# arkworks-rs/circom-compat

Measured on NVIDIA H100. Metric: groth16_proofs_per_sec_bn254_2p20, higher is better.
Workload: dtype u32x8 (254-bit Montgomery integers)

## Files before the change

### circom_compat_b200/csrc/ec.cuh

```cuda
#pragma once
#include "fp.cuh"

namespace b2g {

template <class F>
struct Affine { typename F::elem x, y; };

template <class F>
struct XYZZ { typename F::elem x, y, zz, zzz; };

template <class F>
struct Curve {
    using E = typename F::elem;
    using Aff = Affine<F>;
    using Pt = XYZZ<F>;

    static __device__ __forceinline__ bool aff_is_inf(const Aff& p) { return F::is_zero(p.x) && F::is_zero(p.y); }
    static __device__ __forceinline__ bool is_inf(const Pt& p) { return F::is_zero(p.zz); }
    static __device__ __forceinline__ Pt infinity() { Pt r; r.x = F::zero(); r.y = F::zero(); r.zz = F::zero(); r.zzz = F::zero(); return r; }
    static __device__ __forceinline__ Pt from_affine(const Aff& p) {
        Pt r;
        if (aff_is_inf(p)) return infinity();
        r.x = p.x; r.y = p.y; r.zz = F::one(); r.zzz = F::one();
        return r;
// ... 21 lines not shown
        E v = F::sqr(u);
        E w = F::mul(u, v);
        E s = F::mul(p.x, v);
        E xx = F::sqr(p.x);
        E m = F::add(F::dbl(xx), xx);
        r.x = F::sub(F::sqr(m), F::dbl(s));
        r.y = F::sub(F::mul(m, F::sub(s, r.x)), F::mul(w, p.y));
        r.zz = F::mul(v, p.zz);
        r.zzz = F::mul(w, p.zzz);
        return r;
    }

    static __device__ __forceinline__ void madd(Pt& acc, const Aff& q) {
        if (aff_is_inf(q)) return;
        if (is_inf(acc)) { acc.x = q.x; acc.y = q.y; acc.zz = F::one(); acc.zzz = F::one(); return; }
        E u2 = F::mul(q.x, acc.zz);
        E s2 = F::mul(q.y, acc.zzz);
        E p = F::sub(u2, acc.x);
        E r = F::sub(s2, acc.y);
        if (F::is_zero(p)) {
            if (F::is_zero(r)) acc = dbl_affine(q);
            else acc = infinity();
            return;
        }
        E pp = F::sqr(p);
        E ppp = F::mul(p, pp);
        E qq = F::mul(acc.x, pp);
        E x3 = F::sub(F::sub(F::sqr(r), ppp), F::dbl(qq));
        E y3 = F::mul_sub(r, F::sub(qq, x3), acc.y, ppp);
        acc.x = x3; acc.y = y3;
        acc.zz = F::mul(acc.zz, pp);
        acc.zzz = F::mul(acc.zzz, ppp);
    }

    static __device__ __forceinline__ void add(Pt& acc, const Pt& q) {
        if (is_inf(q)) return;
        if (is_inf(acc)) { acc = q; return; }
        E u1 = F::mul(acc.x, q.zz);
        E u2 = F::mul(q.x, acc.zz);
        E s1 = F::mul(acc.y, q.zzz);
        E s2 = F::mul(q.y, acc.zzz);
        E p = F::sub(u2, u1);
        E r = F::sub(s2, s1);
        if (F::is_zero(p)) {
            if (F::is_zero(r)) acc = dbl(acc);
            else acc = infinity();
            return;
        }
        E pp = F::sqr(p);
        E ppp = F::mul(p, pp);
        E qq = F::mul(u1, pp);
        E x3 = F::sub(F::sub(F::sqr(r), ppp), F::dbl(qq));
        E y3 = F::sub(F::mul(r, F::sub(qq, x3)), F::mul(s1, ppp));
        acc.x = x3; acc.y = y3;
        acc.zz = F::mul(F::mul(acc.zz, q.zz), pp);
        acc.zzz = F::mul(F::mul(acc.zzz, q.zzz), ppp);
    }

    static __device__ __noinline__ Pt mul_scalar(const Pt& p, const uint32_t* k) {
        Pt acc = infinity();
        int top = 255;
        while (top >= 0 && !((k[top >> 5] >> (top & 31)) & 1u)) top--;
        for (int i = top; i >= 0; i--) {
            acc = dbl(acc);
            if ((k[i >> 5] >> (i & 31)) & 1u) add(acc, p);
        }
        return acc;
    }

    static __device__ __noinline__ Aff to_affine(const Pt& p) {
        Aff r;
        if (is_inf(p)) { r.x = F::zero(); r.y = F::zero(); return r; }
        E iz = F::inv(p.zzz);
        r.y = F::mul(p.y, iz);
        E izz = F::mul(F::sqr(p.zz), F::sqr(iz));
        r.x = F::mul(p.x, izz);
        return r;
    }
};

using G1 = Curve<Fq>;
using G2 = Curve<Fq2>;

__device__ __forceinline__ fe curve_b(const Fq*) { fe t = fe_zero(); t.l[0] = 3; return Fq::from_canonical(t); }
__device__ __forceinline__ fe2 curve_b(const Fq2*) {
    fe c0, c1;
    c0.l[0] = 0x24a138e5u; c0.l[1] = 0x3267e6dcu; c0.l[2] = 0x59dbefa3u; c0.l[3] = 0xb5b4c5e5u; c0.l[4] = 0x1be06ac3u; c0.l[5] = 0x81be1899u; c0.l[6] = 0xceb8aaaeu; c0.l[7] = 0x2b149d40u;
    c1.l[0] = 0x85c315d2u; c1.l[1] = 0xe4a2bd06u; c1.l[2] = 0xe52d1852u; c1.l[3] = 0xa74fa084u; c1.l[4] = 0xeed8fdf4u; c1.l[5] = 0xcd2cafadu; c1.l[6] = 0x3af0fed4u; c1.l[7] = 0x009713b0u;
    fe2 r; r.c0 = Fq::from_canonical(c0); r.c1 = Fq::from_canonical(c1);
    return r;
}
template <class C, class F>
__device__ __forceinline__ bool aff_on_curve(const Affine<F>& p) {
    if (C::aff_is_inf(p)) return true;
    typename F::elem lhs = F::sqr(p.y);
    typename F::elem rhs = F::add(F::mul(F::sqr(p.x), p.x), curve_b((const F*)nullptr));
    return F::eq(lhs, rhs);
}

__device__ __forceinline__ void elem_load(fe& r, const void* p) { r = fe_load(p); }
__device__ __forceinline__ void elem_load(fe2& r, const void* p) { r.c0 = fe_load(p); r.c1 = fe_load((const char*)p + 32); }
__device__ __forceinline__ void elem_load_nc(fe& r, const void* p) { r = fe_load_nc(p); }
__device__ __forceinline__ void elem_load_nc(fe2& r, const void* p) { r.c0 = fe_load_nc(p); r.c1 = fe_load_nc((const char*)p + 32); }
__device__ __forceinline__ void elem_store(void* p, const fe& v) { fe_store(p, v); }
__device__ __forceinline__ void elem_store(void* p, const fe2& v) { fe_store(p, v.c0); fe_store((char*)p + 32, v.c1); }

template <class F> struct Bytes;
template <> struct Bytes<Fq> { static constexpr int ELEM = 32; };
template <> struct Bytes<Fq2> { static constexpr int ELEM = 64; };

template <class F>
__device__ __forceinline__ Affine<F> aff_load(const void* base, size_t idx) {
    const char* p = (const char*)base + idx * (2 * Bytes<F>::ELEM);
    Affine<F> r; elem_load_nc(r.x, p); elem_load_nc(r.y, p + Bytes<F>::ELEM);
    return r;
}
template <class F>
__device__ __forceinline__ void aff_store(void* base, size_t idx, const Affine<F>& v) {
    char* p = (char*)base + idx * (2 * Bytes<F>::ELEM);
    elem_store(p, v.x); elem_store(p + Bytes<F>::ELEM, v.y);
}
template <class F>
__device__ __forceinline__ XYZZ<F> pt_load(const void* base, size_t idx) {
    const char* p = (const char*)base + idx * (4 * Bytes<F>::ELEM);
    XYZZ<F> r; elem_load(r.x, p); elem_load(r.y, p + Bytes<F>::ELEM); elem_load(r.zz, p + 2 * Bytes<F>::ELEM); elem_load(r.zzz, p + 3 * Bytes<F>::ELEM);
    return r;
}
template <class F>
__device__ __forceinline__ void pt_store(void* base, size_t idx, const XYZZ<F>& v) {
    char* p = (char*)base + idx * (4 * Bytes<F>::ELEM);
    elem_store(p, v.x); elem_store(p + Bytes<F>::ELEM, v.y); elem_store(p + 2 * Bytes<F>::ELEM, v.zz); elem_store(p + 3 * Bytes<F>::ELEM, v.zzz);
}

}
```

### circom_compat_b200/csrc/fp.cuh

```cuda
#pragma once
#include <cstdint>
#include <cuda_runtime.h>

namespace b2g {

struct alignas(32) fe { uint32_t l[8]; };

struct FqParams {
    static constexpr uint32_t P0 = 0xd87cfd47u, P1 = 0x3c208c16u, P2 = 0x6871ca8du, P3 = 0x97816a91u,
                              P4 = 0x8181585du, P5 = 0xb85045b6u, P6 = 0xe131a029u, P7 = 0x30644e72u;
    static constexpr uint32_t INV = 0xe4866389u;
    static constexpr uint32_t R0 = 0xc58f0d9du, R1 = 0xd35d438du, R2 = 0xf5c70b3du, R3 = 0x0a78eb28u,
                              R4 = 0x7879462cu, R5 = 0x666ea36fu, R6 = 0x9a07df2fu, R7 = 0x0e0a77c1u;
    static constexpr uint32_t RR0 = 0x538afa89u, RR1 = 0xf32cfc5bu, RR2 = 0xd44501fbu, RR3 = 0xb5e71911u,
                              RR4 = 0x0a417ff6u, RR5 = 0x47ab1effu, RR6 = 0xcab8351fu, RR7 = 0x06d89f71u;
};
struct FrParams {
    static constexpr uint32_t P0 = 0xf0000001u, P1 = 0x43e1f593u, P2 = 0x79b97091u, P3 = 0x2833e848u,
                              P4 = 0x8181585du, P5 = 0xb85045b6u, P6 = 0xe131a029u, P7 = 0x30644e72u;
    static constexpr uint32_t INV = 0xefffffffu;
    static constexpr uint32_t R0 = 0x4ffffffbu, R1 = 0xac96341cu, R2 = 0x9f60cd29u, R3 = 0x36fc7695u,
                              R4 = 0x7879462eu, R5 = 0x666ea36fu, R6 = 0x9a07df2fu, R7 = 0x0e0a77c1u;
    static constexpr uint32_t RR0 = 0xae216da7u, RR1 = 0x1bb8e645u, RR2 = 0xe35c59e3u, RR3 = 0x53fe3ab1u,
                              RR4 = 0x53bb8085u, RR5 = 0x8c49833du, RR6 = 0x7f4e44a5u, RR7 = 0x0216d0b1u;
// ... 381 lines not shown
            : "+r"(r.l[0]), "+r"(r.l[1]), "+r"(r.l[2]), "+r"(r.l[3]), "+r"(r.l[4]), "+r"(r.l[5]), "+r"(r.l[6]), "+r"(r.l[7])
            : "r"(t[8]), "r"(t[9]), "r"(t[10]), "r"(t[11]), "r"(t[12]), "r"(t[13]), "r"(t[14]), "r"(t[15]));
        return reduce_once(r);
    }

    static __device__ __forceinline__ void mul_wide_cols(uint32_t* t, const fe& a, const fe& b) {
        uint32_t ev[17], od[16];
        #pragma unroll
        for (int i = 0; i < 17; i++) ev[i] = 0;
        #pragma unroll
        for (int i = 0; i < 16; i++) od[i] = 0;
        #pragma unroll
        for (int i = 0; i < 8; i += 2) {
            cmad4(&ev[i], ev[i + 8], a.l[0], a.l[2], a.l[4], a.l[6], b.l[i]);
            cmad4(&od[i], od[i + 8 < 16 ? i + 8 : 15], a.l[1], a.l[3], a.l[5], a.l[7], b.l[i]);
            cmad4(&od[i], od[i + 8 < 16 ? i + 8 : 15], a.l[0], a.l[2], a.l[4], a.l[6], b.l[i + 1]);
            cmad4(&ev[i + 2], ev[i + 10 < 17 ? i + 10 : 16], a.l[1], a.l[3], a.l[5], a.l[7], b.l[i + 1]);
        }
        t[0] = ev[0];
        asm("add.cc.u32 %0, %15, %30;\n\t"
            "addc.cc.u32 %1, %16, %31;\n\t"
            "addc.cc.u32 %2, %17, %32;\n\t"
            "addc.cc.u32 %3, %18, %33;\n\t"
            "addc.cc.u32 %4, %19, %34;\n\t"
            "addc.cc.u32 %5, %20, %35;\n\t"
            "addc.cc.u32 %6, %21, %36;\n\t"
            "addc.cc.u32 %7, %22, %37;\n\t"
            "addc.cc.u32 %8, %23, %38;\n\t"
            "addc.cc.u32 %9, %24, %39;\n\t"
            "addc.cc.u32 %10, %25, %40;\n\t"
            "addc.cc.u32 %11, %26, %41;\n\t"
            "addc.cc.u32 %12, %27, %42;\n\t"
            "addc.cc.u32 %13, %28, %43;\n\t"
            "addc.u32 %14, %29, %44;"
            : "=r"(t[1]), "=r"(t[2]), "=r"(t[3]), "=r"(t[4]), "=r"(t[5]), "=r"(t[6]), "=r"(t[7]), "=r"(t[8]),
              "=r"(t[9]), "=r"(t[10]), "=r"(t[11]), "=r"(t[12]), "=r"(t[13]), "=r"(t[14]), "=r"(t[15])
            : "r"(ev[1]), "r"(ev[2]), "r"(ev[3]), "r"(ev[4]), "r"(ev[5]), "r"(ev[6]), "r"(ev[7]), "r"(ev[8]),
              "r"(ev[9]), "r"(ev[10]), "r"(ev[11]), "r"(ev[12]), "r"(ev[13]), "r"(ev[14]), "r"(ev[15]),
              "r"(od[0]), "r"(od[1]), "r"(od[2]), "r"(od[3]), "r"(od[4]), "r"(od[5]), "r"(od[6]), "r"(od[7]),
              "r"(od[8]), "r"(od[9]), "r"(od[10]), "r"(od[11]), "r"(od[12]), "r"(od[13]), "r"(od[14]));
    }

    static __device__ __forceinline__ fe mul_sub(const fe& a, const fe& b, const fe& c, const fe& d) {
        uint32_t u[16], v[16];
        mul_wide(u, a, b);
        mul_wide(v, c, d);
        const uint32_t br = sub_wide(u, v);
        add_p_high(u, br);
        return redc(u);
    }

    static __device__ __forceinline__ fe from_canonical(const fe& a) { return mul(a, r2()); }
    static __device__ __forceinline__ fe to_canonical(const fe& a) {
        fe o = fe_zero(); o.l[0] = 1; return mul(a, o);
    }

    static __device__ __noinline__ fe inv(const fe& a) {
        const uint32_t e[8] = {P::P0 - 2u, P::P1, P::P2, P::P3, P::P4, P::P5, P::P6, P::P7};
        fe acc = one();
        for (int i = 255; i >= 0; i--) {
            acc = sqr(acc);
            if ((e[i >> 5] >> (i & 31)) & 1u) acc = mul(acc, a);
        }
        return acc;
    }
};

using Fq = Fp<FqParams>;
using Fr = Fp<FrParams>;

struct fe2 { fe c0, c1; };

#define B2G_FQ2_CALL __noinline__
struct Fq2 {
    using elem = fe2;
    static __device__ __forceinline__ fe2 zero() { fe2 r; r.c0 = fe_zero(); r.c1 = fe_zero(); return r; }
    static __device__ __forceinline__ fe2 one() { fe2 r; r.c0 = Fq::one(); r.c1 = fe_zero(); return r; }
    static __device__ __forceinline__ bool is_zero(const fe2& a) { return fe_is_zero(a.c0) && fe_is_zero(a.c1); }
    static __device__ __forceinline__ bool eq(const fe2& a, const fe2& b) { return fe_equal(a.c0, b.c0) && fe_equal(a.c1, b.c1); }
    static __device__ __forceinline__ fe2 add(const fe2& a, const fe2& b) { fe2 r; r.c0 = Fq::add(a.c0, b.c0); r.c1 = Fq::add(a.c1, b.c1); return r; }
    static __device__ __forceinline__ fe2 sub(const fe2& a, const fe2& b) { fe2 r; r.c0 = Fq::sub(a.c0, b.c0); r.c1 = Fq::sub(a.c1, b.c1); return r; }
    static __device__ __forceinline__ fe2 dbl(const fe2& a) { fe2 r; r.c0 = Fq::dbl(a.c0); r.c1 = Fq::dbl(a.c1); return r; }
    static __device__ __forceinline__ fe2 neg(const fe2& a) { fe2 r; r.c0 = Fq::neg(a.c0); r.c1 = Fq::neg(a.c1); return r; }
    static __device__ B2G_FQ2_CALL fe2 mul(const fe2& a, const fe2& b) {
        uint32_t v0[16], v1[16], v2[16];
        fe sa = add_noreduce(a.c0, a.c1), sb = add_noreduce(b.c0, b.c1);
        Fq::mul_wide_cols(v0, a.c0, b.c0);
        Fq::mul_wide_cols(v1, a.c1, b.c1);
        Fq::mul_wide_cols(v2, sa, sb);
        Fq::sub_wide(v2, v0);
        Fq::sub_wide(v2, v1);
        const uint32_t br = Fq::sub_wide(v0, v1);
        Fq::add_p_high(v0, br);
        fe2 r; r.c0 = Fq::redc(v0); r.c1 = Fq::redc(v2);
        return r;
    }
    static __device__ __forceinline__ fe add_noreduce(const fe& a, const fe& b) {
        fe s;
        asm("add.cc.u32 %0, %8, %16;\n\t"
            "addc.cc.u32 %1, %9, %17;\n\t"
            "addc.cc.u32 %2, %10, %18;\n\t"
            "addc.cc.u32 %3, %11, %19;\n\t"
            "addc.cc.u32 %4, %12, %20;\n\t"
            "addc.cc.u32 %5, %13, %21;\n\t"
            "addc.cc.u32 %6, %14, %22;\n\t"
            "addc.u32 %7, %15, %23;"
            : "=r"(s.l[0]), "=r"(s.l[1]), "=r"(s.l[2]), "=r"(s.l[3]), "=r"(s.l[4]), "=r"(s.l[5]), "=r"(s.l[6]), "=r"(s.l[7])
            : "r"(a.l[0]), "r"(a.l[1]), "r"(a.l[2]), "r"(a.l[3]), "r"(a.l[4]), "r"(a.l[5]), "r"(a.l[6]), "r"(a.l[7]),
              "r"(b.l[0]), "r"(b.l[1]), "r"(b.l[2]), "r"(b.l[3]), "r"(b.l[4]), "r"(b.l[5]), "r"(b.l[6]), "r"(b.l[7]));
        return s;
    }
    static __device__ B2G_FQ2_CALL fe2 mul_sub(const fe2& a, const fe2& b, const fe2& c, const fe2& d) { return sub(mul(a, b), mul(c, d)); }
    static __device__ B2G_FQ2_CALL fe2 sqr(const fe2& a) {
        fe s = Fq::add(a.c0, a.c1), d = Fq::sub(a.c0, a.c1), m = Fq::mul(a.c0, a.c1);
        fe2 r; r.c0 = Fq::mul(s, d); r.c1 = Fq::dbl(m);
        return r;
    }
    static __device__ __noinline__ fe2 inv(const fe2& a) {
        fe d = Fq::inv(Fq::add(Fq::sqr(a.c0), Fq::sqr(a.c1)));
        fe2 r; r.c0 = Fq::mul(a.c0, d); r.c1 = Fq::neg(Fq::mul(a.c1, d));
        return r;
    }
};

}
```

### circom_compat_b200/csrc/msm.cu

```cuda
#include <algorithm>
#include <vector>
#include "msm.cuh"
#include "util.cuh"

namespace b2g {

std::atomic<uint64_t> g_launch_count{0};

template <class C, class F>
__global__ void __launch_bounds__(128) msm_table_kernel(const void* __restrict__ bases, uint32_t n, int c, int nwin, void* __restrict__ table) {
    uint32_t i = blockIdx.x * blockDim.x + threadIdx.x;
    if (i >= n) return;
    using Pt = typename C::Pt; using Aff = typename C::Aff; using E = typename F::elem;
    Aff p = aff_load<F>(bases, i);
    if (C::aff_is_inf(p)) {
        Aff z; z.x = F::zero(); z.y = F::zero();
        for (int w = 0; w < nwin; w++) aff_store<F>(table, (size_t)w * n + i, z);
        return;
    }
    Pt pts[MSM_MAX_WIN];
    E pre[MSM_MAX_WIN];
    Pt cur = C::from_affine(p);
    E acc = F::one();
    for (int w = 0; w < nwin; w++) {
        pts[w] = cur;
        pre[w] = acc;
        acc = F::mul(acc, cur.zzz);
        if (w + 1 < nwin) for (int j = 0; j < c; j++) cur = C::dbl(cur);
    }
    E inv = F::inv(acc);
    for (int w = nwin - 1; w >= 0; w--) {
        E iz = F::mul(inv, pre[w]);
        inv = F::mul(inv, pts[w].zzz);
        Aff a;
        a.y = F::mul(pts[w].y, iz);
        a.x = F::mul(pts[w].x, F::mul(F::sqr(pts[w].zz), F::sqr(iz)));
        aff_store<F>(table, (size_t)w * n + i, a);
    }
}

template <class C, class F>
__global__ void __launch_bounds__(256) msm_validate_kernel(const void* __restrict__ bases, uint32_t n, uint32_t* __restrict__ bad) {
    uint32_t i = blockIdx.x * blockDim.x + threadIdx.x;
    if (i >= n) return;
    if (!aff_on_curve<C, F>(aff_load<F>(bases, i))) atomicMax(bad, i + 1u);
}

__global__ void __launch_bounds__(256) msm_canon_kernel(const fe* __restrict__ scalars, uint32_t n, int scalars_mont, fe* __restrict__ canon_out) {
    uint32_t i = blockIdx.x * blockDim.x + threadIdx.x;
    if (i >= n) return;
    fe k = fe_load_nc(&scalars[i]);
    if (scalars_mont) k = Fr::to_canonical(k);
    fe_store(&canon_out[i], k);
}

__device__ __forceinline__ uint32_t msm_window_bits(const uint32_t* __restrict__ k, int c, int w) {
    const uint32_t off = (uint32_t)w * (uint32_t)c, limb = off >> 5, sh = off & 31u;
    if (limb >= 8) return 0u;
    uint64_t v = __ldg(&k[limb]);
    if (limb + 1 < 8 && sh + (uint32_t)c > 32u) v |= (uint64_t)__ldg(&k[limb + 1]) << 32;
    return (uint32_t)(v >> sh) & ((1u << c) - 1u);
}

__device__ __forceinline__ int32_t msm_digit_at(const uint32_t* __restrict__ k, int c, int w) {
    const uint32_t half = 1u << (c - 1);
    uint32_t carry = 0;
    for (int v = w - 1; v >= 0; v--) {
        const uint32_t b = msm_window_bits(k, c, v);
        if (b >= half) { carry = 1; break; }
        if (b < half - 1) break;
    }
    const uint32_t coef = msm_window_bits(k, c, w) + carry;
    const uint32_t cout = (coef + half) >> c;
    return (int32_t)coef - (int32_t)(cout << c);
}

constexpr int MSM_LEADER_ROUNDS = 2;

__global__ void __launch_bounds__(256) msm_count_kernel(const fe* __restrict__ canon, uint32_t n, int c, int nwin, uint32_t* __restrict__ counts) {
    const uint64_t tid = (uint64_t)blockIdx.x * blockDim.x + threadIdx.x;
    const uint32_t w = (uint32_t)(tid / n), i = (uint32_t)(tid % n);
    int32_t d = 0;
    if (w < (uint32_t)nwin) d = msm_digit_at(canon[i].l, c, (int)w);
// ... 178 lines not shown
    E run = F::one();
    #pragma unroll 1
    for (int i = 0; i < MSM_AFF_M; i++) {
        const uint64_t q64 = (uint64_t)t + (uint64_t)i * stride;
        if (q64 >= total) break;
        const uint32_t q = (uint32_t)q64;
        Aff P, Q; E d;
        const int kind = aff_fetch<C, F, LEVEL0>(table, entries, prev, src[q], P, Q, d);
        if (kind >= AFF_ADD) {
            elem_store((char*)pref + (size_t)q * Bytes<F>::ELEM, run);
            run = F::mul(run, d);
        }
    }
    elem_store((char*)totals + (size_t)t * Bytes<F>::ELEM, run);
}

template <class F>
__global__ void __launch_bounds__(64) msm_aff_invert_kernel(void* __restrict__ totals, void* __restrict__ scratch, uint32_t count, uint32_t U) {
    using E = typename F::elem;
    const uint32_t u = blockIdx.x * blockDim.x + threadIdx.x;
    if (u >= U) return;
    constexpr size_t B = Bytes<F>::ELEM;
    E run = F::one();
    int last = -1;
    #pragma unroll 1
    for (int v = 0; v < MSM_AFF_S; v++) {
        const uint64_t idx = (uint64_t)u + (uint64_t)v * U;
        if (idx >= count) break;
        E x; elem_load(x, (const char*)totals + idx * B);
        elem_store((char*)scratch + idx * B, run);
        run = F::mul(run, x);
        last = v;
    }
    if (last < 0) return;
    E inv = F::inv(run);
    #pragma unroll 1
    for (int v = last; v >= 0; v--) {
        const uint64_t idx = (uint64_t)u + (uint64_t)v * U;
        E x, pre; elem_load(x, (const char*)totals + idx * B); elem_load(pre, (const char*)scratch + idx * B);
        elem_store((char*)totals + idx * B, F::mul(inv, pre));
        inv = F::mul(inv, x);
    }
}

template <class C, class F, bool LEVEL0>
__global__ void __launch_bounds__(128) msm_aff_apply_kernel(const void* __restrict__ table, const uint32_t* __restrict__ entries, const void* __restrict__ prev,
                                                            const uint32_t* __restrict__ src, const uint32_t* __restrict__ off_cur, uint32_t nb,
                                                            const void* __restrict__ pref, const void* __restrict__ totals_inv, void* __restrict__ out) {
    using E = typename F::elem; using Aff = typename C::Aff;
    const uint32_t total = off_cur[nb];
    const uint32_t t = blockIdx.x * blockDim.x + threadIdx.x, stride = gridDim.x * blockDim.x;
    if (t >= total) return;
    E inv; elem_load(inv, (const char*)totals_inv + (size_t)t * Bytes<F>::ELEM);
    int i = MSM_AFF_M - 1;
    while ((uint64_t)t + (uint64_t)i * stride >= total) i--;
    #pragma unroll 1
    for (; i >= 0; i--) {
        const uint32_t q = t + (uint32_t)i * stride;
        Aff P, Q; E d;
        const int kind = aff_fetch<C, F, LEVEL0>(table, entries, prev, src[q], P, Q, d);
        Aff r;
        if (kind >= AFF_ADD) {
            E pre; elem_load(pre, (const char*)pref + (size_t)q * Bytes<F>::ELEM);
            const E inv_d = F::mul(inv, pre);
            inv = F::mul(inv, d);
            E num;
            if (kind == AFF_ADD) num = F::sub(Q.y, P.y);
            else { const E xx = F::sqr(P.x); num = F::add(F::dbl(xx), xx); Q.x = P.x; }
            const E lam = F::mul(num, inv_d);
            r.x = F::sub(F::sub(F::sqr(lam), P.x), Q.x);
            r.y = F::sub(F::mul(lam, F::sub(P.x, r.x)), P.y);
        } else if (kind == AFF_COPY_P) r = P;
        else if (kind == AFF_COPY_Q) r = Q;
        else { r.x = F::zero(); r.y = F::zero(); }
        aff_store<F>(out, (size_t)q, r);
    }
}

template <class F> struct AccOcc;
#ifndef B2G_G1_CTAS
#define B2G_G1_CTAS 4
#endif
template <> struct AccOcc<Fq> { static constexpr int MIN_CTAS = B2G_G1_CTAS; };
#ifndef B2G_G2_CTAS
#define B2G_G2_CTAS 3
#endif
template <> struct AccOcc<Fq2> { static constexpr int MIN_CTAS = B2G_G2_CTAS; };

template <class C, class F>
__global__ void __launch_bounds__(128, AccOcc<F>::MIN_CTAS) msm_accumulate_kernel(const void* __restrict__ table, const uint32_t* __restrict__ entries,
                                      const uint32_t* __restrict__ offsets, uint32_t nb, uint32_t chunk,
                                      void* __restrict__ buckets, void* __restrict__ frag_first, void* __restrict__ frag_last, uint32_t slab_words) {
    using Pt = typename C::Pt; using Aff = typename C::Aff;
    const uint32_t total = offsets[nb];
    const uint32_t t = blockIdx.x * blockDim.x + threadIdx.x;
    const uint64_t start64 = (uint64_t)t * chunk;
    extern __shared__ __align__(128) uint32_t slab[];
    __shared__ __align__(8) unsigned long long slab_bar;
    const uint64_t cta_first = (uint64_t)blockIdx.x * blockDim.x * chunk;
    if (slab_words) {
        const uint32_t bar = (uint32_t)__cvta_generic_to_shared(&slab_bar);
        if (threadIdx.x == 0) {
            asm volatile("mbarrier.init.shared::cta.b64 [%0], 1;" :: "r"(bar));
            asm volatile("fence.mbarrier_init.release.cluster;" ::: "memory");
        }
        __syncthreads();
        if (threadIdx.x == 0 && cta_first < total) {
            const uint64_t left = total - cta_first;
            const uint32_t bytes = (uint32_t)(((left < slab_words ? left : (uint64_t)slab_words) * 4 + 15) & ~15ull);
            asm volatile("mbarrier.arrive.expect_tx.shared::cta.b64 _, [%0], %1;" :: "r"(bar), "r"(bytes) : "memory");
            asm volatile("cp.async.bulk.shared::cluster.global.mbarrier::complete_tx::bytes [%0], [%1], %2, [%3];"
                         :: "r"((uint32_t)__cvta_generic_to_shared(slab)), "l"(entries + cta_first), "r"(bytes), "r"(bar) : "memory");
        }
        if (cta_first < total) {
            uint32_t done = 0;
            while (!done)
                asm volatile("{\n\t.reg .pred p;\n\tmbarrier.try_wait.parity.shared::cta.b64 p, [%1], 0;\n\tselp.u32 %0, 1, 0, p;\n\t}" : "=r"(done) : "r"(bar) : "memory");
        }
    }
    if (start64 >= total) return;
    const uint32_t start = (uint32_t)start64;
    const uint32_t end = (uint32_t)min((uint64_t)total, start64 + chunk);
    uint32_t lo = 0, hi = nb;
    while (hi - lo > 1) { uint32_t mid = (lo + hi) >> 1; if (offsets[mid] <= start) lo = mid; else hi = mid; }
    uint32_t b = lo;
    uint32_t bucket_end = offsets[b + 1];
    while (bucket_end <= start) { b++; bucket_end = offsets[b + 1]; }
    Pt acc = C::infinity();
    uint32_t seg_start = start;
    for (uint32_t pos = start; pos < end;) {
        const uint32_t e = slab_words ? slab[pos - (uint32_t)cta_first] : (entries ? entries[pos] : pos);
        Aff p = aff_load<F>(table, (size_t)(e & 0x7fffffffu));
        if (e >> 31) p.y = F::neg(p.y);
        C::madd(acc, p);
        pos++;
        if (pos == bucket_end || pos == end) {
            const uint32_t bucket_start = offsets[b];
            if (bucket_start >= start && bucket_end <= end) pt_store<F>(buckets, b, acc);
            else if (seg_start == start) pt_store<F>(frag_first, t, acc);
            else pt_store<F>(frag_last, t, acc);
            acc = C::infinity();
            seg_start = pos;
            if (pos == bucket_end && pos < end) {
                do { b++; bucket_end = offsets[b + 1]; } while (bucket_end <= pos);
            }
        }
    }
}


template <class C, class F>
__global__ void __launch_bounds__(128) msm_fold_kernel(const uint32_t* __restrict__ offsets, uint32_t nb, uint32_t chunk, void* __restrict__ buckets,
                                const void* __restrict__ frag_first, const void* __restrict__ frag_last,
                                uint32_t* __restrict__ big_list, uint32_t* __restrict__ big_count) {
    using Pt = typename C::Pt;
    uint32_t b = blockIdx.x * blockDim.x + threadIdx.x;
    if (b >= nb) return;
    uint32_t s = offsets[b], e = offsets[b + 1];
    if (s == e) { pt_store<F>(buckets, b, C::infinity()); return; }
    uint32_t t0 = s / chunk, t1 = (e - 1) / chunk;
    if (t0 == t1) return;
    if (t1 - t0 + 1 > (uint32_t)MSM_BIG_FRAGS) { big_list[atomicAdd(big_count, 1u)] = b; return; }
    Pt acc = (s == t0 * chunk) ? pt_load<F>(frag_first, t0) : pt_load<F>(frag_last, t0);
    for (uint32_t t = t0 + 1; t <= t1; t++) { Pt q = pt_load<F>(frag_first, t); C::add(acc, q); }
    pt_store<F>(buckets, b, acc);
}

template <class F> struct PtWords;
template <> struct PtWords<Fq> { static constexpr int N = 32; };
template <> struct PtWords<Fq2> { static constexpr int N = 64; };

template <class C, class F>
__device__ __forceinline__ typename C::Pt warp_sum_points(typename C::Pt v) {
    using Pt = typename C::Pt;
    static_assert(sizeof(Pt) == PtWords<F>::N * 4, "XYZZ point layout");
    #pragma unroll 1
    for (int d = 16; d > 0; d >>= 1) {
        Pt q;
        uint32_t* qw = reinterpret_cast<uint32_t*>(&q);
        const uint32_t* vw = reinterpret_cast<const uint32_t*>(&v);
        #pragma unroll
        for (int i = 0; i < PtWords<F>::N; i++) qw[i] = __shfl_down_sync(0xffffffffu, vw[i], d);
        if ((int)(threadIdx.x & 31) < d) C::add(v, q);
    }
    return v;
}

template <class C, class F, int NT>
__device__ __forceinline__ typename C::Pt block_sum_points(typename C::Pt v, typename C::Pt* sh) {
    static_assert(NT == 32 || NT == 64, "one or two warps");
    v = warp_sum_points<C, F>(v);
    if (NT == 32) return v;
    if ((threadIdx.x & 31) == 0) sh[threadIdx.x >> 5] = v;
    __syncthreads();
    if (threadIdx.x == 0) { typename C::Pt q = sh[1]; C::add(v, q); }
    __syncthreads();
    return v;
}

template <class F> struct TailThreads;
template <> struct TailThreads<Fq> { static constexpr int N = 64; };
template <> struct TailThreads<Fq2> { static constexpr int N = 32; };
constexpr int MSM_REDUCE_CHUNK_DEFAULT = 8;

template <class C, class F>
__global__ void __launch_bounds__(TailThreads<F>::N) msm_fold_big_kernel(const uint32_t* __restrict__ offsets, uint32_t chunk, void* __restrict__ buckets,
                                    const void* __restrict__ frag_first, const void* __restrict__ frag_last,
                                    const uint32_t* __restrict__ big_list, const uint32_t* __restrict__ big_count) {
    using Pt = typename C::Pt;
    extern __shared__ __align__(32) unsigned char smem_raw[];
    Pt* sh = reinterpret_cast<Pt*>(smem_raw);
    const uint32_t nbig = *big_count;
    for (uint32_t bi = blockIdx.x; bi < nbig; bi += gridDim.x) {
        uint32_t b = big_list[bi];
        uint32_t s = offsets[b], e = offsets[b + 1];
        uint32_t t0 = s / chunk, t1 = (e - 1) / chunk;
        Pt acc = C::infinity();
        for (uint32_t t = t0 + threadIdx.x; t <= t1; t += TailThreads<F>::N) {
            Pt q = (t == t0 && s != t0 * chunk) ? pt_load<F>(frag_last, t0) : pt_load<F>(frag_first, t);
            C::add(acc, q);
        }
        Pt r = block_sum_points<C, F, TailThreads<F>::N>(acc, sh);
        if (threadIdx.x == 0) pt_store<F>(buckets, b, r);
        __syncthreads();
// ... 98 lines not shown
    }
    CUDA_CHECK(cudaMalloc(&s.big_list, (size_t)nbuckets * 4));
    CUDA_CHECK(cudaMalloc(&s.big_count, 4));
    CUDA_CHECK(cudaMalloc(&s.frag_first, nchunks * pt));
    CUDA_CHECK(cudaMalloc(&s.frag_last, nchunks * pt));
    CUDA_CHECK(cudaMalloc(&s.buckets, (size_t)nbuckets * pt));
    CUDA_CHECK(cudaMalloc(&s.partials, (npart + 1) * pt));
    CUDA_CHECK(cudaMalloc(&s.result, pt)); s.result_owned = true;
    {
        int rounds = 0;
        const char* ov = getenv("B2G_MSM_AFFINE_ROUNDS");
        if (ov && *ov) { long x = strtol(ov, nullptr, 10); rounds = x < 0 ? 0 : (x > MSM_AFF_MAX_ROUNDS ? MSM_AFF_MAX_ROUNDS : (int)x); }
        s.aff_cap_rounds = rounds;
        s.aff_nmax[0] = (uint32_t)nent;
        for (int k = 1; k <= rounds; k++) s.aff_nmax[k] = s.aff_nmax[k - 1] / 2 + nbuckets / 2 + 1;
        if (rounds) {
            const size_t elem = g2 ? 64 : 32, aff = 2 * elem;
            if (with_sort) {
                std::vector<uint32_t*> offs(MSM_AFF_MAX_ROUNDS + 1, nullptr);
                offs[0] = s.offsets;
                for (int k = 1; k <= rounds; k++) {
                    CUDA_CHECK(cudaMalloc(&s.aff_off[k], ((size_t)nbuckets + 1) * 4));
                    CUDA_CHECK(cudaMalloc(&s.aff_src[k], ((size_t)s.aff_nmax[k] + 1) * 4));
                    offs[k] = s.aff_off[k];
                }
                s.aff_off[0] = s.offsets;
                CUDA_CHECK(cudaMalloc(&s.aff_off_dev, (MSM_AFF_MAX_ROUNDS + 1) * sizeof(uint32_t*)));
                CUDA_CHECK(cudaMemcpy(s.aff_off_dev, offs.data(), (MSM_AFF_MAX_ROUNDS + 1) * sizeof(uint32_t*), cudaMemcpyHostToDevice));
            }
            CUDA_CHECK(cudaMalloc(&s.aff_list[0], ((size_t)s.aff_nmax[1] + 1) * aff));
            if (rounds > 1) CUDA_CHECK(cudaMalloc(&s.aff_list[1], ((size_t)s.aff_nmax[2] + 1) * aff));
            const size_t threads1 = ((size_t)s.aff_nmax[1] + MSM_AFF_M - 1) / MSM_AFF_M + 128;
            CUDA_CHECK(cudaMalloc(&s.aff_pref, ((size_t)s.aff_nmax[1] + 1) * elem));
            CUDA_CHECK(cudaMalloc(&s.aff_totals, threads1 * elem));
            CUDA_CHECK(cudaMalloc(&s.aff_tscratch, threads1 * elem));
        }
    }
    if (env_u32("B2G_MSM_TAIL_PRIORITY", 1) == 1) {
        int least = 0, greatest = 0;
        CUDA_CHECK(cudaDeviceGetStreamPriorityRange(&least, &greatest));
        CUDA_CHECK(cudaStreamCreateWithPriority(&s.tail, cudaStreamNonBlocking, greatest));
        CUDA_CHECK(cudaEventCreateWithFlags(&s.ev_acc, cudaEventDisableTiming));
        CUDA_CHECK(cudaEventCreateWithFlags(&s.ev_tail, cudaEventDisableTiming));
    }
}

void msm_scratch_free(MsmScratch& s) {
    void* ptrs[] = {s.counts, s.offsets, s.cursor, s.entries, s.big_list, s.big_count, s.frag_first, s.frag_last,
                    s.buckets, s.partials, s.result_owned ? s.result : nullptr, s.scalars_canon,
                    s.aff_list[0], s.aff_list[1], s.aff_pref, s.aff_totals, s.aff_tscratch, s.aff_off_dev};
    for (void* p : ptrs) if (p) cudaFree(p);
    for (int k = 1; k <= MSM_AFF_MAX_ROUNDS; k++) { if (s.aff_off[k]) cudaFree(s.aff_off[k]); if (s.aff_src[k]) cudaFree(s.aff_src[k]); }
    if (s.tail) { cudaStreamDestroy(s.tail); cudaEventDestroy(s.ev_acc); cudaEventDestroy(s.ev_tail); }
    s = MsmScratch();
}

void msm_sort(const MsmPlan& plan, MsmScratch& s, const fe* scalars_dev, uint32_t n, bool scalars_mont, cudaStream_t st) {
    if (n > plan.n) n = plan.n;
    s.sorted_n = n;
    if (n == 0 || plan.table == nullptr) return;
    if (n > s.cap_n || plan.nwin > s.cap_nwin || plan.nbuckets > s.cap_buckets || !s.entries) throw_error(B2G_E_SHAPE, "msm: sort scratch too small");
    const uint32_t nb = plan.nbuckets;
    constexpr unsigned SORT_CTA = 256;
    CUDA_CHECK(cudaMemsetAsync(s.counts, 0, (size_t)nb * 4, st));
    const unsigned pair_blocks = (unsigned)(((uint64_t)n * plan.nwin + SORT_CTA - 1) / SORT_CTA);
    msm_canon_kernel<<<(n + SORT_CTA - 1) / SORT_CTA, SORT_CTA, 0, st>>>(scalars_dev, n, scalars_mont ? 1 : 0, s.scalars_canon);
    msm_count_kernel<<<pair_blocks, SORT_CTA, 0, st>>>(s.scalars_canon, n, plan.c, plan.nwin, s.counts);
    msm_scan_kernel<<<1, 1024, 0, st>>>(s.counts, nb, s.offsets, s.cursor);
    msm_scatter_kernel<<<pair_blocks, SORT_CTA, 0, st>>>(s.scalars_canon, n, plan.n, plan.c, plan.nwin, s.offsets, s.cursor, s.entries);
    g_launch_count += 4;
    s.aff_rounds = s.aff_off_dev ? s.aff_cap_rounds : 0;
    if (s.aff_rounds) {
        msm_aff_levels_kernel<<<1, 1024, 0, st>>>(nb, s.aff_rounds, s.aff_off_dev);
        for (int k = 1; k <= s.aff_rounds; k++) {
            const unsigned blocks = (unsigned)std::min<uint64_t>(((uint64_t)s.aff_nmax[k] + 255) / 256, 1u << 20);
            msm_aff_src_kernel<<<blocks, 256, 0, st>>>(s.aff_off[k - 1], s.aff_off[k], nb, s.aff_src[k]);
        }
        g_launch_count += 1 + s.aff_rounds;
    }
    CUDA_CHECK(cudaGetLastError());
}

template <class C, class F>
static void msm_accumulate_t(const MsmPlan& plan, const MsmScratch& sorted, MsmScratch& s, cudaStream_t st) {
    using Pt = typename C::Pt;
    const size_t ptb = sizeof(Pt);
    const uint32_t n = sorted.sorted_n;
    if (n == 0 || plan.table == nullptr) { CUDA_CHECK(cudaMemsetAsync(s.result, 0, ptb, st)); return; }
    if (plan.nbuckets > s.cap_buckets || n > s.cap_n || plan.nwin > s.cap_nwin) throw_error(B2G_E_SHAPE, "msm: accumulate scratch too small");
    const uint32_t nb = plan.nbuckets, chunk = s.chunk;
    CUDA_CHECK(cudaMemsetAsync(s.big_count, 0, 4, st));
    const uint64_t nent = (uint64_t)n * plan.nwin;
    const uint32_t nthreads = (uint32_t)((nent + chunk - 1) / chunk);
    if (s.prof0) CUDA_CHECK(cudaEventRecord(s.prof0, st));
    int rounds = sorted.aff_rounds < s.aff_cap_rounds ? sorted.aff_rounds : s.aff_cap_rounds;
    if (rounds && (sorted.aff_nmax[1] > s.aff_nmax[1] || !s.aff_list[0])) rounds = 0;
    const uint32_t* offsets = sorted.offsets;
    if (rounds) {
        const void* prev = nullptr;
        for (int k = 1; k <= rounds; k++) {
            const uint32_t nk = sorted.aff_nmax[k];
            const unsigned blocks = (unsigned)(((uint64_t)nk + (uint64_t)MSM_AFF_M * 128 - 1) / ((uint64_t)MSM_AFF_M * 128));
            const uint32_t stride = blocks * 128u, U = (stride + MSM_AFF_S - 1) / MSM_AFF_S;
            void* out = s.aff_list[(k - 1) & 1];
            if (k == 1) {
                msm_aff_prod_kernel<C, F, true><<<blocks, 128, 0, st>>>(plan.table, sorted.entries, nullptr, sorted.aff_src[k], sorted.aff_off[k], nb, s.aff_pref, s.aff_totals);
                msm_aff_invert_kernel<F><<<(U + 63) / 64, 64, 0, st>>>(s.aff_totals, s.aff_tscratch, stride, U);
                msm_aff_apply_kernel<C, F, true><<<blocks, 128, 0, st>>>(plan.table, sorted.entries, nullptr, sorted.aff_src[k], sorted.aff_off[k], nb, s.aff_pref, s.aff_totals, out);
            } else {
                msm_aff_prod_kernel<C, F, false><<<blocks, 128, 0, st>>>(nullptr, nullptr, prev, sorted.aff_src[k], sorted.aff_off[k], nb, s.aff_pref, s.aff_totals);
                msm_aff_invert_kernel<F><<<(U + 63) / 64, 64, 0, st>>>(s.aff_totals, s.aff_tscratch, stride, U);
                msm_aff_apply_kernel<C, F, false><<<blocks, 128, 0, st>>>(nullptr, nullptr, prev, sorted.aff_src[k], sorted.aff_off[k], nb, s.aff_pref, s.aff_totals, out);
            }
            prev = out;
        }
        g_launch_count += 3 * rounds;
        offsets = sorted.aff_off[rounds];
        const uint32_t nthreads_r = (uint32_t)(((uint64_t)sorted.aff_nmax[rounds] + chunk - 1) / chunk);
        msm_accumulate_kernel<C, F><<<(nthreads_r + 127) / 128, 128, 0, st>>>(prev, nullptr, offsets, nb, chunk, s.buckets, s.frag_first, s.frag_last, 0u);
    } else
    {
        static const char* bulk_env = getenv("B2G_ACC_BULK");
        const bool bulk = bulk_env && *bulk_env ? *bulk_env == '1' : !plan.g2;
        const uint32_t slab_words = bulk && (size_t)chunk * 128 * 4 <= 48 * 1024 ? chunk * 128u : 0u;
        msm_accumulate_kernel<C, F><<<(nthreads + 127) / 128, 128, (size_t)slab_words * 4, st>>>(plan.table, sorted.entries, sorted.offsets, nb, chunk, s.buckets, s.frag_first,
                                                                                                  s.frag_last, slab_words);
    }
    if (s.prof1) CUDA_CHECK(cudaEventRecord(s.prof1, st));
    cudaStream_t main_st = st;
    if (s.tail) { CUDA_CHECK(cudaEventRecord(s.ev_acc, st)); CUDA_CHECK(cudaStreamWaitEvent(s.tail, s.ev_acc, 0)); st = s.tail; }
    msm_fold_kernel<C, F><<<(nb + 127) / 128, 128, 0, st>>>(offsets, nb, chunk, s.buckets, s.frag_first, s.frag_last, s.big_list, s.big_count);
    constexpr int NT = TailThreads<F>::N;
    const size_t sh = (size_t)NT * ptb;
    msm_fold_big_kernel<C, F><<<128, NT, sh, st>>>(offsets, chunk, s.buckets, s.frag_first, s.frag_last, s.big_list, s.big_count);
    const uint32_t rchunk = s.reduce_chunk;
    const uint32_t nred = (nb + rchunk - 1) / rchunk;
    const uint32_t npart = (nred + NT - 1) / NT;
    msm_reduce_kernel<C, F><<<npart, NT, sh, st>>>(s.buckets, nb, rchunk, s.partials);
    msm_sum_kernel<C, F><<<1, NT, sh, st>>>(s.partials, npart, s.result);
    if (s.tail) { CUDA_CHECK(cudaEventRecord(s.ev_tail, s.tail)); CUDA_CHECK(cudaStreamWaitEvent(main_st, s.ev_tail, 0)); }
    g_launch_count += 5;
    CUDA_CHECK(cudaGetLastError());
}

void msm_accumulate(const MsmPlan& plan, const MsmScratch& sorted, MsmScratch& acc, cudaStream_t st) {
    if (plan.g2) msm_accumulate_t<G2, Fq2>(plan, sorted, acc, st);
    else msm_accumulate_t<G1, Fq>(plan, sorted, acc, st);
}

void msm_run(const MsmPlan& plan, MsmScratch& s, const fe* scalars_dev, uint32_t n, bool scalars_mont, cudaStream_t st) {
    msm_sort(plan, s, scalars_dev, n, scalars_mont, st);
    msm_accumulate(plan, s, s, st);
}

void msm_init_kernels() {}

}
```

Before: 33.94.

## Split G2 bucket accumulation across thread pairs with shuffle-based mixed addition

Adds a dedicated G2 accumulate kernel in which each bucket run is processed by two cooperating threads. Each thread holds one half of the point (x/zz or y/zzz coordinates) and the two exchange partial products through warp shuffles, so the Fq2 multiplications of a mixed addition are split between them. Fq2 multiply and square get inlined variants for this path. The aim is to cut per-thread register pressure and serial latency in the G2 bucket accumulation, in exchange for shuffle traffic, twice as many threads per run, and branch conditions that both lanes of a pair must agree on.

```diff
diff --git a/circom_compat_b200/csrc/ec.cuh b/circom_compat_b200/csrc/ec.cuh
--- a/circom_compat_b200/csrc/ec.cuh
+++ b/circom_compat_b200/csrc/ec.cuh
@@ -127,6 +127,49 @@
 using G1 = Curve<Fq>;
 using G2 = Curve<Fq2>;
 
+struct G2Pair {
+    static __device__ __forceinline__ void dbl_affine(fe2& s0, fe2& s1, const fe2& qc, bool A, unsigned mask) {
+        const fe2 o1 = Fq2::sel(A, qc, Fq2::dbl(qc));
+        const fe2 sq = Fq2::sqr_inline(o1), sq_o = Fq2::shfl_pair(mask, sq);
+        const fe2 v = Fq2::sel(A, sq_o, sq), xx = Fq2::sel(A, sq, sq_o);
+        const fe2 m2 = Fq2::mul_inline(o1, v), m2_o = Fq2::shfl_pair(mask, m2);
+        const fe2 s = Fq2::sel(A, m2, m2_o), w = Fq2::sel(A, m2_o, m2);
+        const fe2 m = Fq2::add(Fq2::dbl(xx), xx);
+        const fe2 x3 = Fq2::sub(Fq2::sqr_inline(m), Fq2::dbl(s));
+        const fe2 m4 = Fq2::mul_inline(Fq2::sel(A, m, w), Fq2::sel(A, Fq2::sub(s, x3), qc));
+        const fe2 m4_o = Fq2::shfl_pair(mask, m4);
+        s0 = Fq2::sel(A, x3, Fq2::sub(m4_o, m4));
+        s1 = Fq2::sel(A, v, w);
+    }
+
+    static __device__ __forceinline__ void madd(fe2& s0, fe2& s1, bool& empty, const fe2& qc, bool A, unsigned mask) {
+        const bool qz = Fq2::is_zero(qc);
+        const bool qz_o = __shfl_xor_sync(mask, (int)qz, 1) != 0;
+        if (qz && qz_o) return;
+        if (empty) { s0 = qc; s1 = Fq2::one(); empty = false; return; }
+        const fe2 d = Fq2::sub(Fq2::mul_inline(qc, s1), s0);
+        const fe2 d_o = Fq2::shfl_pair(mask, d);
+        const bool z = Fq2::is_zero(d), z_o = Fq2::is_zero(d_o);
+        if (A ? z : z_o) {
+            if (A ? z_o : z) dbl_affine(s0, s1, qc, A, mask);
+            else { s0 = Fq2::zero(); s1 = Fq2::zero(); empty = true; }
+            return;
+        }
+        const fe2 u = Fq2::sel(A, s0, d_o);
+        const fe2 v = Fq2::sel(A, d_o, s0);
+        const fe2 sq = Fq2::sqr_inline(d);
+        const fe2 pp = Fq2::sel(A, sq, Fq2::shfl_pair(mask, sq));
+        const fe2 m3 = Fq2::mul_inline(u, pp);
+        const fe2 rp = Fq2::shfl_pair(mask, Fq2::sub(sq, m3));
+        const fe2 x3 = Fq2::sub(rp, Fq2::dbl(m3));
+        const fe2 b5 = Fq2::sel(A, Fq2::sub(m3, x3), m3);
+        s1 = Fq2::mul_inline(s1, Fq2::sel(A, pp, m3));
+        const fe2 m5 = Fq2::mul_inline(v, b5);
+        const fe2 m5_o = Fq2::shfl_pair(mask, m5);
+        s0 = Fq2::sel(A, x3, Fq2::sub(m5_o, m5));
+    }
+};
+
 __device__ __forceinline__ fe curve_b(const Fq*) { fe t = fe_zero(); t.l[0] = 3; return Fq::from_canonical(t); }
 __device__ __forceinline__ fe2 curve_b(const Fq2*) {
     fe c0, c1;
diff --git a/circom_compat_b200/csrc/fp.cuh b/circom_compat_b200/csrc/fp.cuh
--- a/circom_compat_b200/csrc/fp.cuh
+++ b/circom_compat_b200/csrc/fp.cuh
@@ -487,12 +487,19 @@
     static __device__ __forceinline__ fe2 sub(const fe2& a, const fe2& b) { fe2 r; r.c0 = Fq::sub(a.c0, b.c0); r.c1 = Fq::sub(a.c1, b.c1); return r; }
     static __device__ __forceinline__ fe2 dbl(const fe2& a) { fe2 r; r.c0 = Fq::dbl(a.c0); r.c1 = Fq::dbl(a.c1); return r; }
     static __device__ __forceinline__ fe2 neg(const fe2& a) { fe2 r; r.c0 = Fq::neg(a.c0); r.c1 = Fq::neg(a.c1); return r; }
-    static __device__ B2G_FQ2_CALL fe2 mul(const fe2& a, const fe2& b) {
+    template <bool COLS>
+    static __device__ __forceinline__ fe2 karatsuba(const fe2& a, const fe2& b) {
         uint32_t v0[16], v1[16], v2[16];
         fe sa = add_noreduce(a.c0, a.c1), sb = add_noreduce(b.c0, b.c1);
-        Fq::mul_wide_cols(v0, a.c0, b.c0);
-        Fq::mul_wide_cols(v1, a.c1, b.c1);
-        Fq::mul_wide_cols(v2, sa, sb);
+        if (COLS) {
+            Fq::mul_wide_cols(v0, a.c0, b.c0);
+            Fq::mul_wide_cols(v1, a.c1, b.c1);
+            Fq::mul_wide_cols(v2, sa, sb);
+        } else {
+            Fq::mul_wide(v0, a.c0, b.c0);
+            Fq::mul_wide(v1, a.c1, b.c1);
+            Fq::mul_wide(v2, sa, sb);
+        }
         Fq::sub_wide(v2, v0);
         Fq::sub_wide(v2, v1);
         const uint32_t br = Fq::sub_wide(v0, v1);
@@ -500,6 +507,8 @@
         fe2 r; r.c0 = Fq::redc(v0); r.c1 = Fq::redc(v2);
         return r;
     }
+    static __device__ B2G_FQ2_CALL fe2 mul(const fe2& a, const fe2& b) { return karatsuba<true>(a, b); }
+    static __device__ __forceinline__ fe2 mul_inline(const fe2& a, const fe2& b) { return karatsuba<false>(a, b); }
     static __device__ __forceinline__ fe add_noreduce(const fe& a, const fe& b) {
         fe s;
         asm("add.cc.u32 %0, %8, %16;\n\t"
@@ -516,9 +525,22 @@
         return s;
     }
     static __device__ B2G_FQ2_CALL fe2 mul_sub(const fe2& a, const fe2& b, const fe2& c, const fe2& d) { return sub(mul(a, b), mul(c, d)); }
-    static __device__ B2G_FQ2_CALL fe2 sqr(const fe2& a) {
+    static __device__ __forceinline__ fe2 sqr_inline(const fe2& a) {
         fe s = Fq::add(a.c0, a.c1), d = Fq::sub(a.c0, a.c1), m = Fq::mul(a.c0, a.c1);
         fe2 r; r.c0 = Fq::mul(s, d); r.c1 = Fq::dbl(m);
+        return r;
+    }
+    static __device__ B2G_FQ2_CALL fe2 sqr(const fe2& a) { return sqr_inline(a); }
+    static __device__ __forceinline__ fe2 sel(bool c, const fe2& a, const fe2& b) {
+        fe2 r;
+        #pragma unroll
+        for (int i = 0; i < 8; i++) { r.c0.l[i] = c ? a.c0.l[i] : b.c0.l[i]; r.c1.l[i] = c ? a.c1.l[i] : b.c1.l[i]; }
+        return r;
+    }
+    static __device__ __forceinline__ fe2 shfl_pair(unsigned mask, const fe2& a) {
+        fe2 r;
+        #pragma unroll
+        for (int i = 0; i < 8; i++) { r.c0.l[i] = __shfl_xor_sync(mask, a.c0.l[i], 1); r.c1.l[i] = __shfl_xor_sync(mask, a.c1.l[i], 1); }
         return r;
     }
     static __device__ __noinline__ fe2 inv(const fe2& a) {
diff --git a/circom_compat_b200/csrc/msm.cu b/circom_compat_b200/csrc/msm.cu
--- a/circom_compat_b200/csrc/msm.cu
+++ b/circom_compat_b200/csrc/msm.cu
@@ -1,4 +1,5 @@
 #include <algorithm>
+#include <type_traits>
 #include <vector>
 #include "msm.cuh"
 #include "util.cuh"
@@ -343,10 +344,37 @@
 #define B2G_G1_CTAS 4
 #endif
 template <> struct AccOcc<Fq> { static constexpr int MIN_CTAS = B2G_G1_CTAS; };
-#ifndef B2G_G2_CTAS
-#define B2G_G2_CTAS 3
-#endif
-template <> struct AccOcc<Fq2> { static constexpr int MIN_CTAS = B2G_G2_CTAS; };
+
+__device__ __forceinline__ void acc_stage_slab(uint32_t* slab, unsigned long long* slab_bar, const uint32_t* __restrict__ entries,
+                                               uint64_t cta_first, uint32_t total, uint32_t slab_words) {
+    const uint32_t bar = (uint32_t)__cvta_generic_to_shared(slab_bar);
+    if (threadIdx.x == 0) {
+        asm volatile("mbarrier.init.shared::cta.b64 [%0], 1;" :: "r"(bar));
+        asm volatile("fence.mbarrier_init.release.cluster;" ::: "memory");
+    }
+    __syncthreads();
+    if (threadIdx.x == 0 && cta_first < total) {
+        const uint64_t left = total - cta_first;
+        const uint32_t bytes = (uint32_t)(((left < slab_words ? left : (uint64_t)slab_words) * 4 + 15) & ~15ull);
+        asm volatile("mbarrier.arrive.expect_tx.shared::cta.b64 _, [%0], %1;" :: "r"(bar), "r"(bytes) : "memory");
+        asm volatile("cp.async.bulk.shared::cluster.global.mbarrier::complete_tx::bytes [%0], [%1], %2, [%3];"
+                     :: "r"((uint32_t)__cvta_generic_to_shared(slab)), "l"(entries + cta_first), "r"(bytes), "r"(bar) : "memory");
+    }
+    if (cta_first < total) {
+        uint32_t done = 0;
+        while (!done)
+            asm volatile("{\n\t.reg .pred p;\n\tmbarrier.try_wait.parity.shared::cta.b64 p, [%1], 0;\n\tselp.u32 %0, 1, 0, p;\n\t}" : "=r"(done) : "r"(bar) : "memory");
+    }
+}
+
+__device__ __forceinline__ uint32_t acc_first_bucket(const uint32_t* __restrict__ offsets, uint32_t nb, uint32_t start, uint32_t& bucket_end) {
+    uint32_t lo = 0, hi = nb;
+    while (hi - lo > 1) { uint32_t mid = (lo + hi) >> 1; if (offsets[mid] <= start) lo = mid; else hi = mid; }
+    uint32_t b = lo;
+    bucket_end = offsets[b + 1];
+    while (bucket_end <= start) { b++; bucket_end = offsets[b + 1]; }
+    return b;
+}
 
 template <class C, class F>
 __global__ void __launch_bounds__(128, AccOcc<F>::MIN_CTAS) msm_accumulate_kernel(const void* __restrict__ table, const uint32_t* __restrict__ entries,
@@ -359,34 +387,12 @@
     extern __shared__ __align__(128) uint32_t slab[];
     __shared__ __align__(8) unsigned long long slab_bar;
     const uint64_t cta_first = (uint64_t)blockIdx.x * blockDim.x * chunk;
-    if (slab_words) {
-        const uint32_t bar = (uint32_t)__cvta_generic_to_shared(&slab_bar);
-        if (threadIdx.x == 0) {
-            asm volatile("mbarrier.init.shared::cta.b64 [%0], 1;" :: "r"(bar));
-            asm volatile("fence.mbarrier_init.release.cluster;" ::: "memory");
-        }
-        __syncthreads();
-        if (threadIdx.x == 0 && cta_first < total) {
-            const uint64_t left = total - cta_first;
-            const uint32_t bytes = (uint32_t)(((left < slab_words ? left : (uint64_t)slab_words) * 4 + 15) & ~15ull);
-            asm volatile("mbarrier.arrive.expect_tx.shared::cta.b64 _, [%0], %1;" :: "r"(bar), "r"(bytes) : "memory");
-            asm volatile("cp.async.bulk.shared::cluster.global.mbarrier::complete_tx::bytes [%0], [%1], %2, [%3];"
-                         :: "r"((uint32_t)__cvta_generic_to_shared(slab)), "l"(entries + cta_first), "r"(bytes), "r"(bar) : "memory");
-        }
-        if (cta_first < total) {
-            uint32_t done = 0;
-            while (!done)
-                asm volatile("{\n\t.reg .pred p;\n\tmbarrier.try_wait.parity.shared::cta.b64 p, [%1], 0;\n\tselp.u32 %0, 1, 0, p;\n\t}" : "=r"(done) : "r"(bar) : "memory");
-        }
-    }
+    if (slab_words) acc_stage_slab(slab, &slab_bar, entries, cta_first, total, slab_words);
     if (start64 >= total) return;
     const uint32_t start = (uint32_t)start64;
     const uint32_t end = (uint32_t)min((uint64_t)total, start64 + chunk);
-    uint32_t lo = 0, hi = nb;
-    while (hi - lo > 1) { uint32_t mid = (lo + hi) >> 1; if (offsets[mid] <= start) lo = mid; else hi = mid; }
-    uint32_t b = lo;
-    uint32_t bucket_end = offsets[b + 1];
-    while (bucket_end <= start) { b++; bucket_end = offsets[b + 1]; }
+    uint32_t bucket_end;
+    uint32_t b = acc_first_bucket(offsets, nb, start, bucket_end);
     Pt acc = C::infinity();
     uint32_t seg_start = start;
     for (uint32_t pos = start; pos < end;) {
@@ -401,6 +407,51 @@
             else if (seg_start == start) pt_store<F>(frag_first, t, acc);
             else pt_store<F>(frag_last, t, acc);
             acc = C::infinity();
+            seg_start = pos;
+            if (pos == bucket_end && pos < end) {
+                do { b++; bucket_end = offsets[b + 1]; } while (bucket_end <= pos);
+            }
+        }
+    }
+}
+
+__global__ void __launch_bounds__(128, 3) msm_accumulate_g2_kernel(const void* __restrict__ table, const uint32_t* __restrict__ entries,
+                                      const uint32_t* __restrict__ offsets, uint32_t nb, uint32_t chunk,
+                                      void* __restrict__ buckets, void* __restrict__ frag_first, void* __restrict__ frag_last, uint32_t slab_words) {
+    const uint32_t total = offsets[nb];
+    const uint32_t t = (blockIdx.x * blockDim.x + threadIdx.x) >> 1;
+    const uint32_t half = threadIdx.x & 1u;
+    const bool A = half == 0;
+    const unsigned mask = 3u << (threadIdx.x & 30u);
+    const uint64_t start64 = (uint64_t)t * chunk;
+    extern __shared__ __align__(128) uint32_t slab[];
+    __shared__ __align__(8) unsigned long long slab_bar;
+    const uint64_t cta_first = (uint64_t)blockIdx.x * (blockDim.x / 2) * chunk;
+    if (slab_words) acc_stage_slab(slab, &slab_bar, entries, cta_first, total, slab_words);
+    if (start64 >= total) return;
+    const uint32_t start = (uint32_t)start64;
+    const uint32_t end = (uint32_t)min((uint64_t)total, start64 + chunk);
+    uint32_t bucket_end;
+    uint32_t b = acc_first_bucket(offsets, nb, start, bucket_end);
+    fe2 s0 = Fq2::zero(), s1 = Fq2::zero();
+    bool empty = true;
+    uint32_t seg_start = start;
+    for (uint32_t pos = start; pos < end;) {
+        const uint32_t e = slab_words ? slab[pos - (uint32_t)cta_first] : (entries ? entries[pos] : pos);
+        fe2 qc;
+        elem_load_nc(qc, (const char*)table + (size_t)(e & 0x7fffffffu) * 128 + half * 64);
+        qc = Fq2::sel((e >> 31) && !A, Fq2::neg(qc), qc);
+        G2Pair::madd(s0, s1, empty, qc, A, mask);
+        pos++;
+        if (pos == bucket_end || pos == end) {
+            const uint32_t bucket_start = offsets[b];
+            char* rec;
+            if (bucket_start >= start && bucket_end <= end) rec = (char*)buckets + (size_t)b * 256;
+            else if (seg_start == start) rec = (char*)frag_first + (size_t)t * 256;
+            else rec = (char*)frag_last + (size_t)t * 256;
+            elem_store(rec + half * 64, s0);
+            elem_store(rec + 128 + half * 64, s1);
+            s0 = Fq2::zero(); s1 = Fq2::zero(); empty = true;
             seg_start = pos;
             if (pos == bucket_end && pos < end) {
                 do { b++; bucket_end = offsets[b + 1]; } while (bucket_end <= pos);
@@ -665,6 +716,19 @@
 }
 
 template <class C, class F>
+static void launch_accumulate(const void* table, const uint32_t* entries, const uint32_t* offsets, uint32_t nb, uint32_t chunk, uint32_t nruns,
+                              const MsmScratch& s, bool bulk, cudaStream_t st) {
+    constexpr bool g2 = std::is_same<F, Fq2>::value;
+    constexpr uint32_t runs_per_cta = g2 ? 64u : 128u;
+    const uint32_t slab_words = bulk && (size_t)chunk * runs_per_cta * 4 <= 48 * 1024 ? chunk * runs_per_cta : 0u;
+    const unsigned blocks = (unsigned)(((uint64_t)nruns + runs_per_cta - 1) / runs_per_cta);
+    if constexpr (g2)
+        msm_accumulate_g2_kernel<<<blocks, 128, (size_t)slab_words * 4, st>>>(table, entries, offsets, nb, chunk, s.buckets, s.frag_first, s.frag_last, slab_words);
+    else
+        msm_accumulate_kernel<C, F><<<blocks, 128, (size_t)slab_words * 4, st>>>(table, entries, offsets, nb, chunk, s.buckets, s.frag_first, s.frag_last, slab_words);
+}
+
+template <class C, class F>
 static void msm_accumulate_t(const MsmPlan& plan, const MsmScratch& sorted, MsmScratch& s, cudaStream_t st) {
     using Pt = typename C::Pt;
     const size_t ptb = sizeof(Pt);
@@ -700,14 +764,12 @@
         g_launch_count += 3 * rounds;
         offsets = sorted.aff_off[rounds];
         const uint32_t nthreads_r = (uint32_t)(((uint64_t)sorted.aff_nmax[rounds] + chunk - 1) / chunk);
-        msm_accumulate_kernel<C, F><<<(nthreads_r + 127) / 128, 128, 0, st>>>(prev, nullptr, offsets, nb, chunk, s.buckets, s.frag_first, s.frag_last, 0u);
+        launch_accumulate<C, F>(prev, nullptr, offsets, nb, chunk, nthreads_r, s, false, st);
     } else
     {
         static const char* bulk_env = getenv("B2G_ACC_BULK");
         const bool bulk = bulk_env && *bulk_env ? *bulk_env == '1' : !plan.g2;
-        const uint32_t slab_words = bulk && (size_t)chunk * 128 * 4 <= 48 * 1024 ? chunk * 128u : 0u;
-        msm_accumulate_kernel<C, F><<<(nthreads + 127) / 128, 128, (size_t)slab_words * 4, st>>>(plan.table, sorted.entries, sorted.offsets, nb, chunk, s.buckets, s.frag_first,
-                                                                                                  s.frag_last, slab_words);
+        launch_accumulate<C, F>(plan.table, sorted.entries, sorted.offsets, nb, chunk, nthreads, s, bulk, st);
     }
     if (s.prof1) CUDA_CHECK(cudaEventRecord(s.prof1, st));
     cudaStream_t main_st = st;
```

After: 36.76, median of 6. 1.08x the previous value.
